# microsoft/OmniParser

Hardware: AMD Instinct MI355X
Metric: screenshots/sec end-to-end (detect+caption) @1920x1080 (higher is better)
Workload: dtype f32 (split-f16x3 MFMA)

## Files before the change

### include/omni_amd.h

```cpp
#ifndef OMNI_AMD_H
#define OMNI_AMD_H

#include <stdint.h>
#include <stddef.h>

#ifdef __cplusplus
extern "C" {
#endif

#define OMNI_ABI_VERSION 3

enum { OMNI_F32 = 0, OMNI_F16 = 1 };
enum { OMNI_ACT_NONE = 0, OMNI_ACT_SILU = 1, OMNI_ACT_GELU = 2 };
enum {
  OMNI_OK = 0,
  OMNI_E_ARG = -1,
  OMNI_E_HIP = -2,
  OMNI_E_NODEV = -3
};

const char* omni_last_error(void);
int omni_abi_version(void);
int omni_device_count(void);
int omni_overflow_count(int reset, unsigned long long* count);
// ... 46 lines not shown

#define OMNI_VOCAB_HEADER_BYTES 32
#define OMNI_VOCAB_MAX_NODES 65536
#define OMNI_VOCAB_MAX_LABEL 64
typedef struct omni_vocab_trie {
  int32_t n_nodes;
  int32_t n_edges;
  int32_t longest;
  int32_t reserved[5];
} omni_vocab_trie_t;

#define OMNI_GEN_CTRL_HEADER_BYTES 32
#define OMNI_GEN_CTRL_MAX_BAD 64
#define OMNI_GEN_CTRL_MAX_BAD_LEN 8
typedef struct omni_gen_ctrl {
  float penalty;
  int32_t ngram;
  int32_t min_new_tokens;
  int32_t begin_index;
  int32_t n_bad;
  int32_t bad_stride;
  int32_t reserved[2];
} omni_gen_ctrl_t;

typedef struct omni_cand {
  float x1, y1, x2, y2;
  float score;
  int32_t cls;
  int32_t anchor;
  int32_t pad;
} omni_cand_t;

int omni_op_launch(const omni_op_t* op, void* stream);

typedef struct omni_plan omni_plan_t;
int omni_plan_create(const omni_op_t* ops, int n_ops, omni_plan_t** out);
int omni_plan_run(omni_plan_t* plan, void* stream);
int omni_plan_capture(omni_plan_t* plan, void* stream);
int omni_plan_replay(omni_plan_t* plan, void* stream);
int omni_plan_num_ops(const omni_plan_t* plan);
void omni_plan_destroy(omni_plan_t* plan);

int omni_resample_coeffs(int in_size, int out_size, int filter, int32_t* h_bounds, int32_t* h_coef);

int omni_plan_time(omni_plan_t* plan, void* stream, int iters, float* ms);

int omni_plan_profile(omni_plan_t* plan, void* stream, float* h_ms);

int omni_debug_tile_map(int mtiles, int ntiles, int xcd_n, long long weight_bytes, int bid, int* mt, int* nt, int* grid,
                        int* xcd_n_used);

int omni_debug_conv_cfg(const omni_op_t* op, int out[8]);

int omni_visual_match_cfg(const omni_op_t* op, long long out[4]);

typedef struct omni_model omni_model_t;

int  omni_model_load(const char* bundle_path, omni_model_t** out);
void omni_model_destroy(omni_model_t* model);
int  omni_model_int(const omni_model_t* model, const char* name, long long* value);
int  omni_model_tensor(const omni_model_t* model, const char* name, void** d_ptr, long long* nbytes);
int  omni_model_run(omni_model_t* model, const char* plan_name);

int  omni_detector_create(const char* bundle_path, omni_model_t** out);
int  omni_detector_infer(omni_model_t* det, const uint8_t* images_rgb, int n_images, int on_device, float* h_boxes, float* h_scores,
                         int32_t* h_classes, int32_t* h_counts);

int  omni_captioner_create(const char* bundle_path, omni_model_t** out);
int  omni_captioner_caption(omni_model_t* cap, const uint8_t* image_rgb, int on_device, int img_h, int img_w, const int32_t* h_boxes_px,
                            int n, int32_t* h_ids);

#ifdef __cplusplus
}
#endif
#endif
```

### omniparser_amd/_lib.py

```python
import ctypes
from ctypes import c_char_p, c_float, c_int, c_int32, c_void_p, POINTER, Structure

from . import build as _build


F32, F16 = 0, 1
ACT_NONE, ACT_SILU, ACT_GELU = 0, 1, 2
OP_CONV, OP_AVGPOOL2, OP_MAXPOOL, OP_RESIZE_NEAREST, OP_LETTERBOX, OP_DETECT_DECODE, OP_NMS = 1, 2, 3, 4, 5, 6, 7
OP_DWCONV3, OP_LAYERNORM, OP_ATTN_ROWS, OP_CHAN_ATTN, OP_PROJ_PREP, OP_ASSEMBLE = 8, 9, 10, 11, 12, 13
OP_EMBED_STEP, OP_ATTN_DECODE, OP_GREEDY_STEP, OP_CROP_RESIZE, OP_DWCONV3_LN, OP_SPLIT_CONVERT, OP_GLUE = 14, 15, 16, 17, 18, 19, 20
OP_OVERLAY, OP_PNG_PACK, OP_PNG_DEFLATE, OP_MLP_FUSED, OP_BEAM_STEP = 21, 22, 23, 24, 25
OP_GREEDY_CTRL_STEP = 26
OP_GREEDY_VOCAB_STEP = 27
OP_VISUAL_MATCH = 28
OP_REGION_OCR = 29
OCR_CLASS_STRIP, OCR_CLASS_TEXT, OCR_CLASS_HARD = 1000, 1001, 1002
CAND_BYTES = 32
ABI_VERSION = 3

EXPORTS = [
    "omni_last_error", "omni_abi_version", "omni_device_count", "omni_op_launch",
    "omni_plan_create", "omni_plan_run", "omni_plan_capture", "omni_plan_replay",
    "omni_plan_num_ops", "omni_plan_destroy", "omni_resample_coeffs", "omni_plan_time", "omni_debug_tile_map",
    "omni_debug_conv_cfg",
    "omni_plan_profile",
    "omni_model_load", "omni_model_destroy", "omni_model_int", "omni_model_tensor", "omni_model_run",
    "omni_detector_create", "omni_detector_infer", "omni_captioner_create", "omni_captioner_caption",
    "omni_overflow_count",
    "omni_visual_match_cfg",
]


class OmniOp(Structure):
    _fields_ = [
        ("kind", c_int32),
        ("dtype", c_int32),
        ("p", c_void_p * 8),
        ("i", c_int32 * 32),
        ("f", c_float * 8),
    ]


class OmniError(RuntimeError):
    pass


_lib = None


def lib():
    global _lib
    if _lib is not None:
        return _lib
    path = _build.ensure_built()
    import torch
    _lib = bind(path)
    return _lib


def bind(path):
    L = ctypes.CDLL(str(path))
    missing = [s for s in EXPORTS if not hasattr(L, s)]
    if missing:
        raise OmniError(f"{path} does not export {missing}")
    L.omni_last_error.restype = c_char_p
    L.omni_abi_version.restype = c_int
    L.omni_device_count.restype = c_int
    L.omni_op_launch.argtypes = [POINTER(OmniOp), c_void_p]
    L.omni_op_launch.restype = c_int
    L.omni_plan_create.argtypes = [POINTER(OmniOp), c_int, POINTER(c_void_p)]
    L.omni_plan_create.restype = c_int
    for name in ("omni_plan_run", "omni_plan_capture", "omni_plan_replay"):
        fn = getattr(L, name)
        fn.argtypes = [c_void_p, c_void_p]
        fn.restype = c_int
    L.omni_plan_num_ops.argtypes = [c_void_p]
    L.omni_plan_num_ops.restype = c_int
    L.omni_plan_destroy.argtypes = [c_void_p]
    L.omni_plan_destroy.restype = None
    L.omni_resample_coeffs.argtypes = [c_int, c_int, c_int, POINTER(c_int32), POINTER(c_int32)]
    L.omni_resample_coeffs.restype = c_int
    L.omni_plan_time.argtypes = [c_void_p, c_void_p, c_int, POINTER(c_float)]
    L.omni_plan_time.restype = c_int
    L.omni_plan_profile.argtypes = [c_void_p, c_void_p, POINTER(c_float)]
    L.omni_plan_profile.restype = c_int
    L.omni_debug_tile_map.argtypes = [c_int, c_int, c_int, ctypes.c_longlong, c_int, POINTER(c_int), POINTER(c_int), POINTER(c_int),
                                      POINTER(c_int)]
    L.omni_debug_tile_map.restype = c_int
    L.omni_debug_conv_cfg.argtypes = [POINTER(OmniOp), POINTER(c_int)]
    L.omni_debug_conv_cfg.restype = c_int
    c_ll = ctypes.c_longlong
    for name in ("omni_model_load", "omni_detector_create", "omni_captioner_create"):
        fn = getattr(L, name)
        fn.argtypes = [c_char_p, POINTER(c_void_p)]
        fn.restype = c_int
    L.omni_model_destroy.argtypes = [c_void_p]
    L.omni_model_destroy.restype = None
    L.omni_model_int.argtypes = [c_void_p, c_char_p, POINTER(c_ll)]
    L.omni_model_int.restype = c_int
    L.omni_model_tensor.argtypes = [c_void_p, c_char_p, POINTER(c_void_p), POINTER(c_ll)]
    L.omni_model_tensor.restype = c_int
    L.omni_model_run.argtypes = [c_void_p, c_char_p]
    L.omni_model_run.restype = c_int
    L.omni_detector_infer.argtypes = [c_void_p, c_void_p, c_int, c_int, POINTER(c_float), POINTER(c_float), POINTER(c_int32), POINTER(c_int32)]
    L.omni_detector_infer.restype = c_int
    L.omni_captioner_caption.argtypes = [c_void_p, c_void_p, c_int, c_int, c_int, POINTER(c_int32), c_int, POINTER(c_int32)]
    L.omni_captioner_caption.restype = c_int
    L.omni_overflow_count.argtypes = [c_int, POINTER(ctypes.c_ulonglong)]
    L.omni_overflow_count.restype = c_int
    L.omni_visual_match_cfg.argtypes = [POINTER(OmniOp), POINTER(ctypes.c_longlong)]
    L.omni_visual_match_cfg.restype = c_int
    if L.omni_abi_version() != ABI_VERSION:
        raise OmniError(f"ABI version mismatch: library {L.omni_abi_version()}, host code {ABI_VERSION} (rebuild: python -m omniparser_amd.build)")
    return L


def overflow_count(reset=True) -> int:
    n = ctypes.c_ulonglong(0)
    rc = lib().omni_overflow_count(1 if reset else 0, ctypes.byref(n))
    if rc:
        raise OmniError(lib().omni_last_error().decode())
    return int(n.value)


def gc_after_eviction():
    import gc
    if gc.get_freeze_count():
        gc.unfreeze()
        gc.collect()
        gc.freeze()


def require_device(device, what):
    import torch
    device = torch.device(device or ("cuda" if torch.cuda.is_available() else "cpu"))
    if device.type == "cuda" and not torch.cuda.is_available():
        raise RuntimeError(f"CUDA device requested but unavailable: {device}")
    if device.type != "cuda":
        raise RuntimeError(f"omniparser_amd {what} is the MI355X path and has no CPU fallback; use the reference implementation on CPU")
    if device.index is None:
        device = torch.device("cuda", torch.cuda.current_device())
    return device

# ... 91 lines not shown
        return ms.value

    def profile(self, stream=None):
        arr = (c_float * len(self.ops))()
        check(lib().omni_plan_profile(self._h, _stream_ptr(stream), arr))
        return list(arr)

    def __len__(self):
        return len(self.ops)

    def __del__(self):
        try:
            if self._h:
                lib().omni_plan_destroy(self._h)
                self._h = None
        except Exception:
            pass


def resample_coeffs(in_size: int, out_size: int, filt: int):
    import numpy as np
    k = lib().omni_resample_coeffs(in_size, out_size, filt, None, None)
    if k <= 0:
        check(k)
    bounds = np.zeros((out_size, 2), dtype=np.int32)
    coef = np.zeros((out_size, k), dtype=np.int32)
    rc = lib().omni_resample_coeffs(
        in_size, out_size, filt,
        bounds.ctypes.data_as(POINTER(c_int32)), coef.ctypes.data_as(POINTER(c_int32)))
    if rc <= 0:
        check(rc)
    return bounds, coef


def tile_map(mtiles: int, ntiles: int, bid: int, xcd_n: int = 1, weight_bytes: int = -1):
    mt, nt, grid, used = c_int(), c_int(), c_int(), c_int()
    check(lib().omni_debug_tile_map(mtiles, ntiles, xcd_n, weight_bytes, bid, ctypes.byref(mt), ctypes.byref(nt), ctypes.byref(grid),
                                    ctypes.byref(used)))
    return mt.value, nt.value, grid.value, used.value


CONV_FAMILIES = ("f32", "f16", "split")
CONV_LOADERS = ("generic", "aligned", "pointwise", "row_patch")
CONV_REDUCE = ("none", "reduce_launch", "in_launch_combine")


def conv_cfg(op: OmniOp) -> dict:
    out = (c_int * 8)()
    check(lib().omni_debug_conv_cfg(ctypes.byref(op), out))
    return {"family": CONV_FAMILIES[out[0]], "bm": out[1], "bn": out[2], "rb": out[3], "loader": CONV_LOADERS[out[4]],
            "splits": out[5], "reduce": CONV_REDUCE[out[6]], "waves": out[7]}


class CModel:

    def __init__(self, path, kind):
        h = c_void_p()
        fn = {"detector": lib().omni_detector_create, "captioner": lib().omni_captioner_create, "model": lib().omni_model_load}[kind]
        check(fn(str(path).encode(), ctypes.byref(h)))
        self._h, self.kind = h, kind

    def int(self, name):
        v = ctypes.c_longlong()
        check(lib().omni_model_int(self._h, name.encode(), ctypes.byref(v)))
        return v.value

    def infer(self, images_u8):
        import numpy as np
        n, md = images_u8.shape[0], self.int("max_det")
        im = np.ascontiguousarray(images_u8)
        boxes = np.zeros((n, md, 4), np.float32); scores = np.zeros((n, md), np.float32)
        cls = np.zeros((n, md), np.int32); cnt = np.zeros((n,), np.int32)
        check(lib().omni_detector_infer(self._h, im.ctypes.data_as(c_void_p), n, 0, boxes.ctypes.data_as(POINTER(c_float)),
                                        scores.ctypes.data_as(POINTER(c_float)), cls.ctypes.data_as(POINTER(c_int32)),
                                        cnt.ctypes.data_as(POINTER(c_int32))))
        return boxes, scores, cls, cnt

    def caption(self, image_u8, boxes_px):
        import numpy as np
        im = np.ascontiguousarray(image_u8)
        bx = np.ascontiguousarray(np.asarray(boxes_px, dtype=np.int32).reshape(-1, 4))
        ids = np.zeros((bx.shape[0], self.int("T")), np.int32)
        check(lib().omni_captioner_caption(self._h, im.ctypes.data_as(c_void_p), 0, im.shape[0], im.shape[1],
                                           bx.ctypes.data_as(POINTER(c_int32)), bx.shape[0], ids.ctypes.data_as(POINTER(c_int32))))
        return ids

    def tensor(self, name):
        p, n = c_void_p(), ctypes.c_longlong()
        check(lib().omni_model_tensor(self._h, name.encode(), ctypes.byref(p), ctypes.byref(n)))
        return p.value, n.value

    def close(self):
        if self._h:
            lib().omni_model_destroy(self._h)
            self._h = None

    def __del__(self):
        try:
            self.close()
        except Exception:
            pass
```

### omniparser_amd/csrc/caption_ops.hip

```cpp
#include "omni_internal.h"
#include <stdlib.h>

#pragma clang fp contract(off)

OMNI_RANGE_GUARD_TU()

namespace {

template <typename T> __device__ __forceinline__ float ldf(const T* p) { return ElemTraits<T>::to_f32(*p); }
template <typename T> __device__ __forceinline__ void stf(T* p, float v) { *p = ElemTraits<T>::from_f32(v); }

__device__ __forceinline__ float wave_sum(float v) {
#pragma unroll
  for (int o = 32; o > 0; o >>= 1) v += __shfl_xor(v, o);
  return v;
}
__device__ __forceinline__ float wave_max(float v) {
#pragma unroll
  for (int o = 32; o > 0; o >>= 1) v = fmaxf(v, __shfl_xor(v, o));
  return v;
}

struct DwArgs { const void* x; const void* w; const float* bias; void* y; int B, H, W, C; long long total; };

template <typename T>
__host__ __device__ __forceinline__ void dwconv3_point_body(const DwArgs& a, long long idx) {
  constexpr int V = ElemTraits<T>::kVec;
  struct Vec { T v[V]; };
  const T* __restrict__ X = (const T*)a.x;
  const T* __restrict__ Wt = (const T*)a.w;
  T* __restrict__ Y = (T*)a.y;
  const int cv = a.C / V;
  int c = (int)(idx % cv) * V;
  long long pix = idx / cv;
  int w = (int)(pix % a.W);
  long long t = pix / a.W;
  int h = (int)(t % a.H);
  long long b = t / a.H;
  float acc[V];
#pragma unroll
  for (int e = 0; e < V; ++e) acc[e] = 0.0f;
  Vec ctr;
#pragma unroll
  for (int r = 0; r < 3; ++r) {
    int hi = h + r - 1;
    if (hi < 0 || hi >= a.H) continue;
#pragma unroll
    for (int s = 0; s < 3; ++s) {
      int wi = w + s - 1;
      if (wi < 0 || wi >= a.W) continue;
      Vec xv = __builtin_bit_cast(Vec, *reinterpret_cast<const u32x4*>(X + ((b * a.H + hi) * a.W + wi) * a.C + c));
      Vec wv = __builtin_bit_cast(Vec, *reinterpret_cast<const u32x4*>(Wt + (r * 3 + s) * a.C + c));
      if (r == 1 && s == 1) ctr = xv;
#pragma unroll
// ... 346 lines not shown
  load_row(h0, r1);
  load_row(h0 + 1, r2);
  const float invC = 1.0f / (float)a.C;
  for (int h = h0; h < h1; ++h) {
    if (h + 1 < h1) load_row(h + 2, nx);
    f32x4 y[NV];
    float s = 0.0f;
#pragma unroll
    for (int i = 0; i < NV; ++i) {
      f32x4 acc = z4;
#pragma unroll
      for (int q = 0; q < 3; ++q) acc += wt[0 + q][i] * r0[q][i];
#pragma unroll
      for (int q = 0; q < 3; ++q) acc += wt[3 + q][i] * r1[q][i];
#pragma unroll
      for (int q = 0; q < 3; ++q) acc += wt[6 + q][i] * r2[q][i];
      y[i] = (acc + cb[i]) + r1[1][i];
      s += (y[i][0] + y[i][1]) + (y[i][2] + y[i][3]);
    }
    const long long pix = (long long)h * a.W + w;
#pragma unroll
    for (int i = 0; i < NV; ++i) *reinterpret_cast<f32x4*>(Y1 + pix * a.C + (l + i * LPP) * 4) = y[i];
    const float mean = group_sum<LPP>(s) * invC;
    float q2 = 0.0f;
#pragma unroll
    for (int i = 0; i < NV; ++i) {
      const f32x4 d = y[i] - mean;
      q2 += (d[0] * d[0] + d[1] * d[1]) + (d[2] * d[2] + d[3] * d[3]);
    }
    const float rstd = 1.0f / sqrtf(group_sum<LPP>(q2) * invC + a.eps);
#pragma unroll
    for (int i = 0; i < NV; ++i) {
      const int c = (l + i * LPP) * 4;
      float o[4];
#pragma unroll
      for (int e = 0; e < 4; ++e) o[e] = (y[i][e] - mean) * rstd * lg[i][e] + lb[i][e];
      if constexpr (OSPLIT) {
        uint2 hi, lo;
        omni_split4(o, hi, lo);
        unsigned char* p = Hh + pix * a.C * 4 + omni_split_off(c);
        *reinterpret_cast<uint2*>(p) = hi;
        *reinterpret_cast<uint2*>(p + 32) = lo;
      } else {
        *reinterpret_cast<f32x4*>(Hh + (pix * a.C + c) * 4) = f32x4{o[0], o[1], o[2], o[3]};
      }
    }
#pragma unroll
    for (int q = 0; q < 3; ++q)
#pragma unroll
      for (int i = 0; i < NV; ++i) { r0[q][i] = r1[q][i]; r1[q][i] = r2[q][i]; r2[q][i] = nx[q][i]; }
  }
}

template <int NV, int LPP>
void launch_dwln_strip(const DwLnArgs& a, hipStream_t s) {
  constexpr int PPB = 256 / LPP;
  const int pxb = (a.W + PPB - 1) / PPB;
  int SR = 16;
  while (SR > 4 && (long long)a.B * ((a.H + SR - 1) / SR) * pxb < 1024) SR >>= 1;
  const int strips = (a.H + SR - 1) / SR;
  const long long nb = (long long)a.B * strips * pxb;
  const unsigned grid = (unsigned)(((nb + 7) / 8) * 8);
  if (a.osplit) hipLaunchKernelGGL((dwln_strip_kernel<NV, LPP, true>), dim3(grid), dim3(256), 0, s, a, SR, pxb, strips, (unsigned)nb);
  else hipLaunchKernelGGL((dwln_strip_kernel<NV, LPP, false>), dim3(grid), dim3(256), 0, s, a, SR, pxb, strips, (unsigned)nb);
}

struct AttnArgs {
  const void* q; const void* k; const void* v; void* o; const float* kbias; const float* vbias;
  int ldq, ldk, ldv, ldo, qoff, koff, voff, ooff;
  int heads, nq, nk, groups;
  int mode, H, W, wy, wx;
  float scale;
  int osplit;
  const int* nkeys;
};

__device__ __forceinline__ int attn_valid_keys(const AttnArgs& a, int g) {
  return a.nkeys ? min(max(a.nkeys[g], 1), a.nk) : a.nk;
}

template <typename T>
__device__ __forceinline__ void store_out(void* base, long long row, int ld, int c, float v, int osplit) {
  if (osplit) {
    unsigned short hi, lo;
    omni_split1(v, hi, lo);
    unsigned short* p = (unsigned short*)base + row * ld * 2 + omni_split_half_index(c);
    p[0] = hi;
    p[16] = lo;
  } else {
    stf((T*)base + row * ld + c, v);
  }
}

__device__ __forceinline__ long long window_row(const AttnArgs& a, int g, int i) {
  int wpi = a.wy * a.wx;
  int b = g / wpi, wrem = g - b * wpi;
  int wyi = wrem / a.wx, wxi = wrem - wyi * a.wx;
  int r = wyi * 12 + i / 12, c = wxi * 12 + i % 12;
  if (r >= a.H || c >= a.W) return -1;
  return ((long long)b * a.H + r) * a.W + c;
}

template <typename T, int D, int NT>
__global__ __launch_bounds__(NT) void attn_rows_kernel(AttnArgs a) {
  constexpr int KT = 48;
  __shared__ __attribute__((aligned(16))) float sk[KT][D];
  __shared__ __attribute__((aligned(16))) float sv[KT][D];
  const int g = blockIdx.z, h = blockIdx.y;
  const int qi = blockIdx.x * NT + threadIdx.x;
  const T* Q = (const T*)a.q; const T* K = (const T*)a.k; const T* V = (const T*)a.v;
  long long qrow = -1;
  if (qi < a.nq) qrow = a.mode == 1 ? window_row(a, g, qi) : (long long)g * a.nq + qi;
  float q[D], o[D];
#pragma unroll
// ... 197 lines not shown
#pragma unroll
      for (int dt = 0; dt < 2; ++dt) {
        const unsigned char* vr = Vh + (dt * 16 + qc) * VROW + (32 * j + 4 * grp) * 2;
        h16x4 a0 = *reinterpret_cast<const h16x4*>(vr), a1 = *reinterpret_cast<const h16x4*>(vr + 32);
        h16x4 b0 = *reinterpret_cast<const h16x4*>(vr + D * VROW), b1 = *reinterpret_cast<const h16x4*>(vr + D * VROW + 32);
        h16x8 vh = {a0[0], a0[1], a0[2], a0[3], a1[0], a1[1], a1[2], a1[3]};
        h16x8 vl = {b0[0], b0[1], b0[2], b0[3], b1[0], b1[1], b1[2], b1[3]};
        oM[dt] = __builtin_amdgcn_mfma_f32_16x16x32_f16(ph, vh, oM[dt], 0, 0, 0);
        oC[dt] = __builtin_amdgcn_mfma_f32_16x16x32_f16(ph, vl, oC[dt], 0, 0, 0);
        oC[dt] = __builtin_amdgcn_mfma_f32_16x16x32_f16(pl, vh, oC[dt], 0, 0, 0);
      }
    }
#pragma unroll
    for (int r = 0; r < 4; ++r) {
      int ql_ = grp * 4 + r;
      float rs = __shfl(sum, ql_);
      long long orow = window_row(a, g, qt * 16 + ql_);
      if (orow >= 0) {
        float inv = 1.0f / rs;
#pragma unroll
        for (int dt = 0; dt < 2; ++dt)
          store_out<T>(a.o, orow, a.ldo, a.ooff + h * D + dt * 16 + qc, (oM[dt][r] + oC[dt][r] * inv2048) * inv, a.osplit);
      }
    }
  }
}

__device__ __forceinline__ void split2(float a, float b, unsigned& h, unsigned& l) {
  typedef __fp16 hv2 __attribute__((ext_vector_type(2)));
  const hv2 hh = __builtin_amdgcn_cvt_pkrtz(a, b);
  const f32x2 r = (f32x2{a, b} - f32x2{(float)hh[0], (float)hh[1]}) * 2048.0f;
  const hv2 ll = __builtin_amdgcn_cvt_pkrtz(r[0], r[1]);
  h = __builtin_bit_cast(unsigned, hh);
  l = __builtin_bit_cast(unsigned, ll);
}
__device__ __forceinline__ void split4v(const f32x4& v, uint2& h, uint2& l) {
  split2(v[0], v[1], h.x, l.x);
  split2(v[2], v[3], h.y, l.y);
}

__device__ __forceinline__ void split2m(float a, float b, unsigned& h, unsigned& l) {
  typedef __fp16 hv2 __attribute__((ext_vector_type(2)));
  const hv2 hh = __builtin_amdgcn_cvt_pkrtz(a, b);
  const f32x2 s = f32x2{a, b} * 2048.0f;
  const hv2 ll = __builtin_amdgcn_cvt_pkrtz(__builtin_fmaf((float)hh[0], -2048.0f, s[0]), __builtin_fmaf((float)hh[1], -2048.0f, s[1]));
  h = __builtin_bit_cast(unsigned, hh);
  l = __builtin_bit_cast(unsigned, ll);
}
__device__ __forceinline__ void split4m(const f32x4& v, uint2& h, uint2& l) {
  split2m(v[0], v[1], h.x, l.x);
  split2m(v[2], v[3], h.y, l.y);
}

__global__ __launch_bounds__(192, 2) void window_attn_mfma_f32_kernel(AttnArgs a) {
  constexpr int D = 32, NKP = 160, KROW = 80, VROW = 336;
  __shared__ __attribute__((aligned(16))) unsigned char lds[2 * NKP * KROW + 2 * D * VROW];
  unsigned char* Kh = lds;
  unsigned char* Kl = lds + NKP * KROW;
  unsigned char* Vh = lds + 2 * NKP * KROW;
  unsigned char* Vl = Vh + D * VROW;
  const int g = blockIdx.z, h = blockIdx.y;
  const int tid = threadIdx.x, lane = tid & 63, wave = tid >> 6;
  const int wpi = a.wy * a.wx;
  const int b = g / wpi, wrem = g - b * wpi;
  const int wyi = wrem / a.wx, wxi = wrem - wyi * a.wx;
  const int r0 = wyi * 12, c0 = wxi * 12;
  const int rows_left = a.H - r0, cols_left = a.W - c0;
  const long long row00 = ((long long)b * a.H + r0) * a.W + c0;
  const float* Qb = (const float*)a.q + row00 * a.ldq + a.qoff + h * D;
  const float* Kb = (const float*)a.k + row00 * a.ldk + a.koff + h * D;
  const float* Vb = (const float*)a.v + row00 * a.ldv + a.voff + h * D;
  const int qc = lane & 15, grp = lane >> 4;
  const f32x4 z4 = {0.f, 0.f, 0.f, 0.f};
  const int iq0 = 16 * wave + qc;
  const int qwr = iq0 / 12, qwc = iq0 - 12 * qwr;
  const int qtok = qwr * a.W + qwc;
  f32x4 qraw[3][2];
#pragma unroll
  for (int t = 0; t < 3; ++t) {
    const bool ok = qwr + 4 * t < rows_left && qwc < cols_left;
    const float* qp = Qb + (ok ? (qtok + 4 * t * a.W) * a.ldq : 0) + grp * 8;
    qraw[t][0] = ok ? *reinterpret_cast<const f32x4*>(qp) : z4;
    qraw[t][1] = ok ? *reinterpret_cast<const f32x4*>(qp + 4) : z4;
  }
  const int t8 = tid >> 3, d0 = (tid & 7) * 4;
  const int kwr = t8 >= 12 ? 1 : 0, kwc = t8 - 12 * kwr;
  const int ktok = kwr * a.W + kwc;
  f32x4 kpad = z4, vpad = z4;
  if (a.kbias) kpad = *reinterpret_cast<const f32x4*>(a.kbias + h * D + d0);
  if (a.vbias) vpad = *reinterpret_cast<const f32x4*>(a.vbias + h * D + d0);
  f32x4 kraw[6];
#pragma unroll
  for (int j = 0; j < 6; ++j) {
    const bool ok = kwr + 2 * j < rows_left && kwc < cols_left;
    kraw[j] = ok ? *reinterpret_cast<const f32x4*>(Kb + (ktok + 2 * j * a.W) * a.ldk + d0) : kpad;
  }
  const int vwr = t8 / 3, vwc = 4 * (t8 - 3 * vwr);
  const int vtok = vwr * a.W + vwc;
  f32x4 vraw[2][4];
#pragma unroll
  for (int j = 0; j < 2; ++j) {
    if (j == 0 || tid < 96) {
#pragma unroll
      for (int u = 0; u < 4; ++u) {
        const bool ok = vwr + 8 * j < rows_left && vwc + u < cols_left;
        vraw[j][u] = ok ? *reinterpret_cast<const f32x4*>(Vb + (vtok + 8 * j * a.W + u) * a.ldv + d0) : vpad;
      }
    }
  }
#pragma unroll
  for (int j = 0; j < 6; ++j) {
    const int key = t8 + 24 * j;
    uint2 kh, kl;
    split4m(kraw[j], kh, kl);
    *reinterpret_cast<uint2*>(Kh + key * KROW + d0 * 2) = kh;
    *reinterpret_cast<uint2*>(Kl + key * KROW + d0 * 2) = kl;
  }
  if (tid >= 128) {
    const int r = tid - 128;
    unsigned char* p = (r < 32 ? Vh : Vl) + (r & 31) * VROW + 144 * 2;
    const u32x4 z = {0u, 0u, 0u, 0u};
    *reinterpret_cast<u32x4*>(p) = z;
    *reinterpret_cast<u32x4*>(p + 16) = z;
  }
#pragma unroll
  for (int j = 0; j < 2; ++j) {
    const int kq = t8 + 24 * j;
    if (j == 0 || tid < 96) {
#pragma unroll
      for (int dd = 0; dd < 4; ++dd) {
        uint2 vh, vl;
        split4m(f32x4{vraw[j][0][dd], vraw[j][1][dd], vraw[j][2][dd], vraw[j][3][dd]}, vh, vl);
        *reinterpret_cast<uint2*>(Vh + (d0 + dd) * VROW + kq * 8) = vh;
        *reinterpret_cast<uint2*>(Vl + (d0 + dd) * VROW + kq * 8) = vl;
      }
    }
  }
  __syncthreads();

  const float inv2048 = 1.0f / 2048.0f;
  const float qscale = a.scale * 1.4426950408889634f;
  unsigned char* const Ob = (unsigned char*)a.o + (row00 * a.ldo + a.ooff + h * D) * 4;
#pragma unroll
  for (int t = 0; t < 3; ++t) {
    u32x4 qhu, qlu;
    {
      const f32x4 q0 = qraw[t][0] * qscale, q1 = qraw[t][1] * qscale;
      uint2 h0, l0, h1, l1;
      split4m(q0, h0, l0);
      split4m(q1, h1, l1);
      qhu = u32x4{h0.x, h0.y, h1.x, h1.y};
      qlu = u32x4{l0.x, l0.y, l1.x, l1.y};
    }
    const h16x8 qh = __builtin_bit_cast(h16x8, qhu), ql = __builtin_bit_cast(h16x8, qlu);
    f32x2 sc[18];
    float mx = -INFINITY;
#pragma unroll
    for (int kt = 0; kt < 9; ++kt) {
      const unsigned char* kr = Kh + (kt * 16 + qc) * KROW + grp * 16;
      const h16x8 kh = *reinterpret_cast<const h16x8*>(kr);
      const h16x8 kl = *reinterpret_cast<const h16x8*>(kr + NKP * KROW);
      f32x4 accM = z4, accC = z4;
      accM = __builtin_amdgcn_mfma_f32_16x16x32_f16(kh, qh, accM, 0, 0, 0);
      accC = __builtin_amdgcn_mfma_f32_16x16x32_f16(kh, ql, accC, 0, 0, 0);
      accC = __builtin_amdgcn_mfma_f32_16x16x32_f16(kl, qh, accC, 0, 0, 0);
      sc[2 * kt] = f32x2{accC[0], accC[1]} * inv2048 + f32x2{accM[0], accM[1]};
      sc[2 * kt + 1] = f32x2{accC[2], accC[3]} * inv2048 + f32x2{accM[2], accM[3]};
      mx = fmaxf(fmaxf(mx, sc[2 * kt][0]), sc[2 * kt][1]);
      mx = fmaxf(fmaxf(mx, sc[2 * kt + 1][0]), sc[2 * kt + 1][1]);
    }
    mx = fmaxf(mx, __shfl_xor(mx, 16));
    mx = fmaxf(mx, __shfl_xor(mx, 32));
    f32x2 sum2 = {0.f, 0.f};
#pragma unroll
    for (int e = 0; e < 18; ++e) {
      const f32x2 d = sc[e] - mx;
      sc[e] = f32x2{__builtin_amdgcn_exp2f(d[0]), __builtin_amdgcn_exp2f(d[1])};
      sum2 += sc[e];
    }
    float sum = sum2[0] + sum2[1];
    sum += __shfl_xor(sum, 16);
    sum += __shfl_xor(sum, 32);
    f32x4 oM[2], oC[2];
#pragma unroll
    for (int dt = 0; dt < 2; ++dt) { oM[dt] = z4; oC[dt] = z4; }
#pragma unroll
    for (int j = 0; j < 5; ++j) {
      unsigned h0, l0, h1, l1, h2 = 0u, l2 = 0u, h3 = 0u, l3 = 0u;
      split2m(sc[4 * j][0], sc[4 * j][1], h0, l0);
      split2m(sc[4 * j + 1][0], sc[4 * j + 1][1], h1, l1);
      if (j < 4) {
        split2m(sc[4 * j + 2][0], sc[4 * j + 2][1], h2, l2);
        split2m(sc[4 * j + 3][0], sc[4 * j + 3][1], h3, l3);
      }
      const h16x8 ph = __builtin_bit_cast(h16x8, u32x4{h0, h1, h2, h3});
      const h16x8 pl = __builtin_bit_cast(h16x8, u32x4{l0, l1, l2, l3});
#pragma unroll
      for (int dt = 0; dt < 2; ++dt) {
        const unsigned char* vr = Vh + (dt * 16 + qc) * VROW + (32 * j + 4 * grp) * 2;
        const uint2 a0 = *reinterpret_cast<const uint2*>(vr), a1 = *reinterpret_cast<const uint2*>(vr + 32);
        const uint2 b0 = *reinterpret_cast<const uint2*>(vr + D * VROW), b1 = *reinterpret_cast<const uint2*>(vr + D * VROW + 32);
        const h16x8 vh = __builtin_bit_cast(h16x8, u32x4{a0.x, a0.y, a1.x, a1.y});
        const h16x8 vl = __builtin_bit_cast(h16x8, u32x4{b0.x, b0.y, b1.x, b1.y});
        oM[dt] = __builtin_amdgcn_mfma_f32_16x16x32_f16(vh, ph, oM[dt], 0, 0, 0);
        oC[dt] = __builtin_amdgcn_mfma_f32_16x16x32_f16(vl, ph, oC[dt], 0, 0, 0);
        oC[dt] = __builtin_amdgcn_mfma_f32_16x16x32_f16(vh, pl, oC[dt], 0, 0, 0);
      }
    }
    if (qwr + 4 * t < rows_left && qwc < cols_left) {
      const float inv = 1.0f / sum;
      unsigned char* orow = Ob + (long long)(qtok + 4 * t * a.W) * a.ldo * 4;
#pragma unroll
      for (int dt = 0; dt < 2; ++dt) {
        const f32x4 o = (oC[dt] * inv2048 + oM[dt]) * inv;
        const int c = dt * 16 + 4 * grp;
        if (a.osplit) {
          const float v[4] = {o[0], o[1], o[2], o[3]};
          uint2 hi, lo;
          omni_split4(v, hi, lo);
          *reinterpret_cast<uint2*>(orow + omni_split_off(c)) = hi;
          *reinterpret_cast<uint2*>(orow + omni_split_off(c) + 32) = lo;
        } else {
          *reinterpret_cast<f32x4*>(orow + c * 4) = o;
        }
      }
    }
  }
}

template <typename T>
__global__ __launch_bounds__(256, 2) void mha_mfma_kernel(AttnArgs a) {
  constexpr int D = 64, KB = 32;
  constexpr int KROW = 144;
  constexpr int VROW = 80;
  __shared__ __attribute__((aligned(16))) unsigned char lds[2 * KB * KROW + 2 * D * VROW];
  unsigned char* Kh = lds;
  unsigned char* Kl = lds + KB * KROW;
  unsigned char* Vh = lds + 2 * KB * KROW;
  unsigned char* Vl = Vh + D * VROW;
  const int g = blockIdx.z, h = blockIdx.y;
  const int tid = threadIdx.x, lane = tid & 63, wave = tid >> 6;
  const int qc = lane & 15, grp = lane >> 4;
  const T* Qp = (const T*)a.q; const T* Kp = (const T*)a.k; const T* Vp = (const T*)a.v;
  const float inv2048 = 1.0f / 2048.0f;

  const int q0 = blockIdx.x * 128 + wave * 32;
  h16x8 qh[2][2], ql[2][2];
#pragma unroll
  for (int t = 0; t < 2; ++t) {
    int qi = q0 + t * 16 + qc;
#pragma unroll
    for (int ks = 0; ks < 2; ++ks) {
#pragma unroll
      for (int u = 0; u < 8; ++u) {
// ... 1593 lines not shown
    for (int y = 0; y < cnt; ++y) {
      const unsigned char* s = a.tmp + (((long long)crop * 64 + ymin + y) * a.R + xx) * 3;
      int kk = k[y]; s0 += s[0] * kk; s1 += s[1] * kk; s2 += s[2] * kk;
    }
    p[0] = clip8b(s0); p[1] = clip8b(s1); p[2] = clip8b(s2);
  }
  T* out = (T*)a.y + ((long long)crop * a.R * a.R + idx) * a.ldo;
#pragma unroll
  for (int c = 0; c < 3; ++c) {
    float v = a.lut[p[c]];
    stf(out + c, (v - a.mean[c]) / a.stdv[c]);
  }
  for (int c = 3; c < a.ldo; ++c) stf(out + c, 0.0f);
}

template <typename F32, typename F16>
int by_dtype(int dtype, const char* name, F32 f32, F16 f16) {
  if (dtype == OMNI_F32) f32();
  else if (dtype == OMNI_F16) f16();
  else { omni_set_error("%s: bad dtype %d", name, dtype); return OMNI_E_ARG; }
  return OMNI_OK;
}

template <typename L>
int by_dtype_scores(int dtype, bool scores, const char* name, L launch) {
  return scores ? by_dtype(dtype, name, [&] { launch(float{}, std::true_type{}); }, [&] { launch(half_t{}, std::true_type{}); })
                : by_dtype(dtype, name, [&] { launch(float{}, std::false_type{}); }, [&] { launch(half_t{}, std::false_type{}); });
}

}

int omni_launch_dwconv3(const omni_op_t* op, hipStream_t s) {
  DwArgs a{};
  a.x = op->p[0]; a.w = op->p[1]; a.bias = (const float*)op->p[2]; a.y = op->p[4];
  a.B = op->i[0]; a.H = op->i[1]; a.W = op->i[2]; a.C = op->i[3];
  OMNI_REQUIRE(a.x && a.w && a.bias && a.y && a.B > 0 && a.H > 0 && a.W > 0 && a.C > 0, "dwconv3: bad arguments");
  OMNI_REQUIRE(a.C % (op->dtype == OMNI_F32 ? 4 : 8) == 0, "dwconv3: C must be a multiple of the 16-byte vector width");
  a.total = (long long)a.B * a.H * a.W * a.C;
  const int V = op->dtype == OMNI_F32 ? 4 : 8;
  const DwStripGrid g = dwconv3_strip_grid(a, V);
  int rc;
  if (g.ok) {
    rc = by_dtype(op->dtype, "dwconv3",
        [&] { hipLaunchKernelGGL(dwconv3_strip_kernel<float>, dim3(g.gx, g.gy, g.gz), dim3(256), 0, s, a, g.cv_log2); },
        [&] { hipLaunchKernelGGL(dwconv3_strip_kernel<half_t>, dim3(g.gx, g.gy, g.gz), dim3(256), 0, s, a, g.cv_log2); });
  } else {
    long long blocks = (a.total / V + 255) / 256; if (blocks > 65536) blocks = 65536;
    rc = by_dtype(op->dtype, "dwconv3",
        [&] { hipLaunchKernelGGL(dwconv3_kernel<float>, dim3((unsigned)blocks), dim3(256), 0, s, a); },
        [&] { hipLaunchKernelGGL(dwconv3_kernel<half_t>, dim3((unsigned)blocks), dim3(256), 0, s, a); });
  }
  if (rc) return rc;
  OMNI_HIP_CHECK(hipGetLastError());
  return OMNI_OK;
}

int omni_launch_dwconv3_ln(const omni_op_t* op, hipStream_t s) {
  DwLnArgs a{};
  a.x = op->p[0]; a.w = op->p[1]; a.bias = (const float*)op->p[2]; a.h = op->p[3]; a.y1 = op->p[4];
  a.g = (const float*)op->p[5]; a.b = (const float*)op->p[6];
  a.B = op->i[0]; a.H = op->i[1]; a.W = op->i[2]; a.C = op->i[3]; a.eps = op->f[0]; a.osplit = op->i[6];
  const int V = op->dtype == OMNI_F32 ? 4 : 8;
  OMNI_REQUIRE(a.x && a.w && a.bias && a.h && a.y1 && a.g && a.b, "dwconv3_ln: null pointer");
  OMNI_REQUIRE(!a.osplit || (op->dtype == OMNI_F32 && a.C % 16 == 0), "dwconv3_ln: split output needs an f32 plan and C %% 16 == 0");
  OMNI_REQUIRE(a.B > 0 && a.H > 0 && a.W > 0 && a.C > 0 && a.C <= 1024 && a.C % V == 0, "dwconv3_ln: bad shape (C <= 1024, C %% %d == 0)", V);
  a.pixels = (long long)a.B * a.H * a.W;
  if (op->dtype == OMNI_F32 && (a.C == 128 || a.C == 256 || a.C == 512) && (long long)a.B * a.H * a.W < (1ll << 31)) {
    if (a.C == 128) launch_dwln_strip<1, 32>(a, s);
    else if (a.C == 256) launch_dwln_strip<1, 64>(a, s);
    else launch_dwln_strip<2, 64>(a, s);
    OMNI_HIP_CHECK(hipGetLastError());
    return OMNI_OK;
  }
  unsigned blocks = (unsigned)((a.pixels + 3) / 4);
  int rc = by_dtype(op->dtype, "dwconv3_ln",
      [&] { hipLaunchKernelGGL(dwconv3_ln_kernel<float>, dim3(blocks), dim3(256), 0, s, a); },
      [&] { hipLaunchKernelGGL(dwconv3_ln_kernel<half_t>, dim3(blocks), dim3(256), 0, s, a); });
  if (rc) return rc;
  OMNI_HIP_CHECK(hipGetLastError());
  return OMNI_OK;
}

int omni_launch_layernorm(const omni_op_t* op, hipStream_t s) {
  LnArgs a{};
  a.x = op->p[0]; a.add = op->p[1]; a.g = (const float*)op->p[2]; a.b = (const float*)op->p[3]; a.y = op->p[4];
  a.rows = ((long long)op->i[0]) * (op->i[1] > 0 ? op->i[1] : 1); a.C = op->i[3]; a.period = op->i[5] > 0 ? op->i[5] : 1;
  a.eps = op->f[0];
  a.omode = op->i[6]; a.y2 = op->p[5];
  OMNI_REQUIRE(a.x && a.g && a.b && a.y && a.rows > 0 && a.C > 0 && a.C <= 1024, "layernorm: bad arguments (C <= 1024)");
  OMNI_REQUIRE(a.omode >= 0 && a.omode <= 2 && (a.omode != 2 || a.y2), "layernorm: bad output mode %d", a.omode);
  OMNI_REQUIRE(a.omode == 0 || (op->dtype == OMNI_F32 && a.C % 16 == 0), "layernorm: split output needs an f32 plan and C %% 16 == 0");
  if (op->dtype == OMNI_F32 && launch_layernorm_v4(a, s)) {
    OMNI_HIP_CHECK(hipGetLastError());
    return OMNI_OK;
  }
  unsigned blocks = (unsigned)((a.rows + 3) / 4);
  int rc = by_dtype(op->dtype, "layernorm",
      [&] { launch_layernorm_typed<float>(a, blocks, s); },
      [&] { launch_layernorm_typed<half_t>(a, blocks, s); });
  if (rc) return rc;
  OMNI_HIP_CHECK(hipGetLastError());
  return OMNI_OK;
}

static int launch_attn_rows(const omni_op_t* op, hipStream_t s) {
  AttnArgs a{};
  a.q = op->p[0]; a.k = op->p[1]; a.v = op->p[2]; a.o = op->p[4];
  a.kbias = (const float*)op->p[5]; a.vbias = (const float*)op->p[6];
  a.ldq = op->i[0]; a.ldk = op->i[1]; a.ldv = op->i[2]; a.ldo = op->i[3];
  a.qoff = op->i[4]; a.koff = op->i[5]; a.voff = op->i[6]; a.ooff = op->i[7];
  a.heads = op->i[8]; a.nq = op->i[9]; a.nk = op->i[10]; a.groups = op->i[11];
  a.mode = op->i[12]; a.H = op->i[13]; a.W = op->i[14];
  int D = op->i[15];
  a.scale = op->f[0];
  a.osplit = op->i[16];
  a.nkeys = (const int*)op->p[7];
  OMNI_REQUIRE(a.q && a.k && a.v && a.o && a.heads > 0 && a.nq > 0 && a.nk > 0 && a.groups > 0, "attn_rows: bad arguments");
  OMNI_REQUIRE(!a.nkeys || a.mode == 0, "attn_rows: the per-group key count (p7) is for mode 0");
  OMNI_REQUIRE(!a.osplit || (op->dtype == OMNI_F32 && a.ldo % 16 == 0 && a.ooff % 16 == 0), "attn_rows: split output needs an f32 plan, 16-channel aligned");
  OMNI_REQUIRE(D == 32 || D == 64, "attn_rows: head_dim %d unsupported", D);
  if (a.mode == 1) {
    OMNI_REQUIRE(a.nq == 144 && a.nk == 144 && a.H > 0 && a.W > 0, "attn_rows: window mode needs 12x12 windows");
    a.wy = (a.H + 11) / 12; a.wx = (a.W + 11) / 12;
    OMNI_REQUIRE(a.groups % (a.wy * a.wx) == 0, "attn_rows: groups must be B * windows");
  } else { a.wy = a.wx = 0; }
  int rc;
  const bool aligned4 = a.ldq % 4 == 0 && a.ldk % 4 == 0 && a.ldv % 4 == 0 && a.ldo % 4 == 0 &&
                        a.qoff % 4 == 0 && a.koff % 4 == 0 && a.voff % 4 == 0 && a.ooff % 4 == 0;
  OMNI_REQUIRE(!a.osplit || (a.mode == 1 && D == 32) || (a.mode == 0 && D == 64), "attn_rows: split output exists on the MFMA kernels only");
  if (a.mode == 1 && D == 32) {
    dim3 grid(1, a.heads, a.groups);
    OMNI_REQUIRE(op->dtype != OMNI_F32 || aligned4, "attn_rows: the f32 window kernel reads 16-byte rows (pitches and channel offsets %% 4 == 0)");
    rc = by_dtype(op->dtype, "attn_rows",
      [&] { hipLaunchKernelGGL(window_attn_mfma_f32_kernel, grid, dim3(192), 0, s, a); },
      [&] { hipLaunchKernelGGL((window_attn_mfma_kernel<half_t>), grid, dim3(192), 0, s, a); });
  } else if (a.mode == 0 && D == 64) {
    dim3 grid((a.nq + 127) / 128, a.heads, a.groups);
    OMNI_REQUIRE(op->dtype != OMNI_F32 || aligned4, "attn_rows: the f32 MHA kernel reads 16-byte rows (pitches and channel offsets %% 4 == 0)");
    rc = by_dtype(op->dtype, "attn_rows",
      [&] { hipLaunchKernelGGL(mha_mfma_f32_kernel, grid, dim3(256), 0, s, a); },
      [&] { hipLaunchKernelGGL((mha_mfma_kernel<half_t>), grid, dim3(256), 0, s, a); });
  } else {
    dim3 grid((a.nq + 127) / 128, a.heads, a.groups);
    if (D == 32) rc = by_dtype(op->dtype, "attn_rows",
      [&] { hipLaunchKernelGGL((attn_rows_kernel<float, 32, 128>), grid, dim3(128), 0, s, a); },
      [&] { hipLaunchKernelGGL((attn_rows_kernel<half_t, 32, 128>), grid, dim3(128), 0, s, a); });
    else rc = by_dtype(op->dtype, "attn_rows",
      [&] { hipLaunchKernelGGL((attn_rows_kernel<float, 64, 128>), grid, dim3(128), 0, s, a); },
      [&] { hipLaunchKernelGGL((attn_rows_kernel<half_t, 64, 128>), grid, dim3(128), 0, s, a); });
  }
  if (rc) return rc;
  OMNI_HIP_CHECK(hipGetLastError());
  return OMNI_OK;
}

int omni_launch_chan_repack(const omni_op_t* op, hipStream_t s) {
  FoldArgs f{};
  const int B = op->i[0], C = op->i[3];
  f.wf = (float*)op->p[0]; f.wb = (unsigned char*)op->p[4]; f.bmax = (float*)op->p[5]; f.osc = (float*)op->p[6];
  OMNI_REQUIRE(op->dtype == OMNI_F32 && f.wf && f.wb && f.bmax && f.osc, "split_convert (i6 = 1): f32 plans, p0 / p4 / p5 / p6");
  OMNI_REQUIRE(B > 0 && C > 0 && C % 64 == 0 && op->i[1] == C && op->i[4] == C && op->i[5] == 0 && op->i[13] == C && op->i[14] == 0,
               "split_convert (i6 = 1): i0 square matrices of i1 = i3 = i4 = i13 = C, C %% 64 == 0, no channel offsets (C %d)", C);
  f.C = C; f.G = C / 32; f.nblk = (C / 64) * (C / 32); f.oscmul = 1.0f;
  hipLaunchKernelGGL(chan_fold_max_kernel, dim3(f.nblk, B), dim3(256), 0, s, f);
  hipLaunchKernelGGL(chan_fold_pack_kernel, dim3((C * (C / 16) + 255) / 256, B), dim3(256), 0, s, f);
  OMNI_HIP_CHECK(hipGetLastError());
  return OMNI_OK;
}

static int launch_chan_attn(const omni_op_t* op, hipStream_t s) {
  ChanArgs a{};
  a.qkv = op->p[0]; a.o = op->p[4]; a.ws = (float*)op->p[5];
  a.B = op->i[0]; a.N = op->i[1]; a.C = op->i[3]; a.G = op->i[4]; a.chunk_tokens = op->i[5]; a.osplit = op->i[6];
  const bool fold = op->i[8] == 1;
  OMNI_REQUIRE(a.qkv && (a.o || fold) && a.ws && a.B > 0 && a.N > 0 && a.C == a.G * 32 && a.chunk_tokens > 0, "chan_attn: bad arguments");
  OMNI_REQUIRE(op->i[8] == 0 || fold, "chan_attn: unknown mode %d", op->i[8]);
  OMNI_REQUIRE(!fold || (op->dtype == OMNI_F32 && a.chunk_tokens % 8 == 0 && a.C % 64 == 0 && op->p[1] && op->p[2] && op->p[3] && op->p[6] && op->p[7]),
               "chan_attn: fold mode needs an f32 plan, C %% 64 == 0, chunk_tokens %% 8 == 0 and p1 / p2 / p3 / p6 / p7");
  OMNI_REQUIRE(!a.osplit || op->dtype == OMNI_F32, "chan_attn: split output needs an f32 plan");
  const int vfold = op->i[11];
  OMNI_REQUIRE(vfold == 0 || (vfold == 1 && fold && a.C % 128 == 0), "chan_attn: i11 = %d needs fold mode (i8 = 1) and C %% 128 == 0, and is 0 or 1", vfold);
  const bool have_scores = op->i[9] == 1;
  if (op->i[10] != 0) {
    OMNI_REQUIRE(op->i[10] > 0 && op->i[10] % 8 == 0 && a.chunk_tokens % op->i[10] == 0 && op->dtype == OMNI_F32 && a.C % 4 == 0,
                 "chan_attn: i10 = %d (tokens per partial) needs an f32 plan, i10 %% 8 == 0 and i5 %% i10 == 0", op->i[10]);
    a.chunk_tokens = op->i[10];
  }
// ... 244 lines not shown
```

Before: 12.91.

## Swizzle window-attention LDS layout and pick dwconv-LN strip height by cost

The f32 window-attention kernel gets a new default LDS layout: K and V split images are XOR-swizzled instead of padded. This shrinks shared memory so three blocks per CU fit instead of two, and it drops the zero-fill of the V pad. Separately, the dwconv3+LN strip launcher for C=128 now picks the strip height from a cost model that uses occupancy-derived slot counts, rather than the fixed 16-row rule. Env vars can force the old paths, and a debug export reports the strip choice. The risks are bank-conflict regressions from the swizzle and extra conditional V reads in the last key chunk.

```diff
diff --git a/include/omni_amd.h b/include/omni_amd.h
--- a/include/omni_amd.h
+++ b/include/omni_amd.h
@@ -122,6 +122,8 @@
 
 int omni_debug_conv_cfg(const omni_op_t* op, int out[8]);
 
+int omni_debug_dwln_sr(const omni_op_t* op, int slots, int out[8]);
+
 int omni_visual_match_cfg(const omni_op_t* op, long long out[4]);
 
 typedef struct omni_model omni_model_t;
diff --git a/omniparser_amd/_lib.py b/omniparser_amd/_lib.py
--- a/omniparser_amd/_lib.py
+++ b/omniparser_amd/_lib.py
@@ -22,7 +22,7 @@
     "omni_last_error", "omni_abi_version", "omni_device_count", "omni_op_launch",
     "omni_plan_create", "omni_plan_run", "omni_plan_capture", "omni_plan_replay",
     "omni_plan_num_ops", "omni_plan_destroy", "omni_resample_coeffs", "omni_plan_time", "omni_debug_tile_map",
-    "omni_debug_conv_cfg",
+    "omni_debug_conv_cfg", "omni_debug_dwln_sr",
     "omni_plan_profile",
     "omni_model_load", "omni_model_destroy", "omni_model_int", "omni_model_tensor", "omni_model_run",
     "omni_detector_create", "omni_detector_infer", "omni_captioner_create", "omni_captioner_caption",
@@ -89,6 +89,8 @@
     L.omni_debug_tile_map.restype = c_int
     L.omni_debug_conv_cfg.argtypes = [POINTER(OmniOp), POINTER(c_int)]
     L.omni_debug_conv_cfg.restype = c_int
+    L.omni_debug_dwln_sr.argtypes = [POINTER(OmniOp), c_int, POINTER(c_int)]
+    L.omni_debug_dwln_sr.restype = c_int
     c_ll = ctypes.c_longlong
     for name in ("omni_model_load", "omni_detector_create", "omni_captioner_create"):
         fn = getattr(L, name)
@@ -286,6 +288,13 @@
             "splits": out[5], "reduce": CONV_REDUCE[out[6]], "waves": out[7]}
 
 
+def dwln_sr(op: OmniOp, slots: int) -> dict:
+    out = (c_int * 8)()
+    check(lib().omni_debug_dwln_sr(ctypes.byref(op), slots, out))
+    return {"sr": out[0], "strips": out[1], "blocks": out[2], "cost_sr": out[3], "cost_rounds": out[4], "cost": out[5],
+            "how": ("rule16", "cost", "forced")[out[6]], "cols_per_block": out[7]}
+
+
 class CModel:
 
     def __init__(self, path, kind):
diff --git a/omniparser_amd/csrc/caption_ops.hip b/omniparser_amd/csrc/caption_ops.hip
--- a/omniparser_amd/csrc/caption_ops.hip
+++ b/omniparser_amd/csrc/caption_ops.hip
@@ -1,5 +1,6 @@
 #include "omni_internal.h"
 #include <stdlib.h>
+#include <string.h>
 
 #pragma clang fp contract(off)
 
@@ -452,14 +453,69 @@
   }
 }
 
+struct DwlnStripCfg { int SR, strips; long long nb; int cost_SR; long long cost_rounds, cost; int how; };
+
+static long long dwln_strip_cost(int B, int H, int pxb, int SR, int slots, long long* rounds) {
+  const int rows = SR < H ? SR : H, strips = (H + rows - 1) / rows;
+  const long long nb = (long long)B * strips * pxb;
+  *rounds = (nb + slots - 1) / slots;
+  const int loaded = rows + (strips == 1 ? 0 : strips == 2 ? 1 : 2);
+  return *rounds * (loaded + 2 * rows);
+}
+
+static bool dwln_cost_adopted(int C) { return C == 128; }
+
+static DwlnStripCfg dwln_strip_cfg(const DwLnArgs& a, int pxb, int slots) {
+  DwlnStripCfg c{};
+  c.cost_SR = 0;
+  if (slots > 0) {
+    const int cand[7] = {8, 16, 24, 32, 48, 96, a.H};
+    for (int k = 0; k < 7; ++k) {
+      if (cand[k] > a.H) continue;
+      long long r;
+      const long long cost = dwln_strip_cost(a.B, a.H, pxb, cand[k], slots, &r);
+      if (!c.cost_SR || cost <= c.cost) { c.cost_SR = cand[k]; c.cost = cost; c.cost_rounds = r; }
+    }
+  }
+  const char* e = getenv("OMNI_DWLN_SR");
+  const bool want_cost = e && !strcmp(e, "cost");
+  const int forced = (e && !want_cost) ? atoi(e) : 0;
+  if (forced > 0) { c.SR = forced < a.H ? forced : a.H; c.how = 2; }
+  else if (c.cost_SR && (want_cost || dwln_cost_adopted(a.C))) { c.SR = c.cost_SR; c.how = 1; }
+  else {
+    c.SR = 16; c.how = 0;
+    while (c.SR > 4 && (long long)a.B * ((a.H + c.SR - 1) / c.SR) * pxb < 1024) c.SR >>= 1;
+  }
+  c.strips = (a.H + c.SR - 1) / c.SR;
+  c.nb = (long long)a.B * c.strips * pxb;
+  return c;
+}
+
+template <int NV, int LPP>
+int dwln_strip_slots() {
+#if defined(__HIP__)
+  static const int slots = [] {
+    int per_cu = 0, dev = 0, cus = 0;
+    if (hipOccupancyMaxActiveBlocksPerMultiprocessor(&per_cu, dwln_strip_kernel<NV, LPP, true>, 256, 0) != hipSuccess ||
+        hipGetDevice(&dev) != hipSuccess || hipDeviceGetAttribute(&cus, hipDeviceAttributeMultiprocessorCount, dev) != hipSuccess) {
+      (void)hipGetLastError();
+      return 0;
+    }
+    return per_cu > 0 && cus > 0 ? per_cu * cus : 0;
+  }();
+  return slots;
+#else
+  return 0;
+#endif
+}
+
 template <int NV, int LPP>
 void launch_dwln_strip(const DwLnArgs& a, hipStream_t s) {
   constexpr int PPB = 256 / LPP;
   const int pxb = (a.W + PPB - 1) / PPB;
-  int SR = 16;
-  while (SR > 4 && (long long)a.B * ((a.H + SR - 1) / SR) * pxb < 1024) SR >>= 1;
-  const int strips = (a.H + SR - 1) / SR;
-  const long long nb = (long long)a.B * strips * pxb;
+  const DwlnStripCfg cfg = dwln_strip_cfg(a, pxb, dwln_strip_slots<NV, LPP>());
+  const int SR = cfg.SR, strips = cfg.strips;
+  const long long nb = cfg.nb;
   const unsigned grid = (unsigned)(((nb + 7) / 8) * 8);
   if (a.osplit) hipLaunchKernelGGL((dwln_strip_kernel<NV, LPP, true>), dim3(grid), dim3(256), 0, s, a, SR, pxb, strips, (unsigned)nb);
   else hipLaunchKernelGGL((dwln_strip_kernel<NV, LPP, false>), dim3(grid), dim3(256), 0, s, a, SR, pxb, strips, (unsigned)nb);
@@ -763,13 +819,34 @@
   split2m(v[2], v[3], h.y, l.y);
 }
 
-__global__ __launch_bounds__(192, 2) void window_attn_mfma_f32_kernel(AttnArgs a) {
-  constexpr int D = 32, NKP = 160, KROW = 80, VROW = 336;
-  __shared__ __attribute__((aligned(16))) unsigned char lds[2 * NKP * KROW + 2 * D * VROW];
+template <bool PADDED> struct WinLds;
+template <> struct WinLds<true> {
+  static constexpr int KIMG = 160 * 80, VIMG = 32 * 336;
+  static __device__ __forceinline__ int k_store(int key, int d0) { return key * 80 + d0 * 2; }
+  static __device__ __forceinline__ int k_read(int kt, int qc, int grp) { return (kt * 16 + qc) * 80 + grp * 16; }
+  static __device__ __forceinline__ int v_chunk(int ch, int c, int lo) { return lo * VIMG + ch * 336 + c * 8; }
+};
+template <> struct WinLds<false> {
+  static constexpr int KIMG = 144 * 64, VIMG = 9 * 1024;
+  static __device__ __forceinline__ int kswz(int key) { return (-(key >> 2)) & 3; }
+  static __device__ __forceinline__ int k_store(int key, int d0) { return key * 64 + (((d0 >> 3) ^ kswz(key)) << 4) + ((d0 & 4) << 1); }
+  static __device__ __forceinline__ int k_read(int kt, int qc, int grp) { return (kt * 16 + qc) * 64 + ((grp ^ kswz(qc)) << 4); }
+  static __device__ __forceinline__ int v_chunk(int ch, int c, int lo) {
+    const int vrow = ((ch >> 2) & 3) | ((ch & 3) << 2) | (ch & 16), vswz = (ch & 1) | ((((ch >> 1) ^ (ch >> 4)) & 1) << 1);
+    const int kb = c >> 2, blk = kb < 8 ? lo * 8 + kb : 16 + lo;
+    return blk * 1024 + vrow * 32 + (((c & 3) ^ vswz) << 3);
+  }
+};
+
+template <bool PADDED>
+__global__ __launch_bounds__(192, PADDED ? 2 : 3) void window_attn_mfma_f32_kernel(AttnArgs a) {
+  constexpr int D = 32;
+  constexpr int KIMG = WinLds<PADDED>::KIMG, VIMG = WinLds<PADDED>::VIMG;
+  typedef WinLds<PADDED> Lds;
+  __shared__ __attribute__((aligned(16))) unsigned char lds[2 * KIMG + 2 * VIMG];
   unsigned char* Kh = lds;
-  unsigned char* Kl = lds + NKP * KROW;
-  unsigned char* Vh = lds + 2 * NKP * KROW;
-  unsigned char* Vl = Vh + D * VROW;
+  unsigned char* Kl = lds + KIMG;
+  unsigned char* V = lds + 2 * KIMG;
   const int g = blockIdx.z, h = blockIdx.y;
   const int tid = threadIdx.x, lane = tid & 63, wave = tid >> 6;
   const int wpi = a.wy * a.wx;
@@ -824,15 +901,18 @@
     const int key = t8 + 24 * j;
     uint2 kh, kl;
     split4m(kraw[j], kh, kl);
-    *reinterpret_cast<uint2*>(Kh + key * KROW + d0 * 2) = kh;
-    *reinterpret_cast<uint2*>(Kl + key * KROW + d0 * 2) = kl;
-  }
-  if (tid >= 128) {
-    const int r = tid - 128;
-    unsigned char* p = (r < 32 ? Vh : Vl) + (r & 31) * VROW + 144 * 2;
-    const u32x4 z = {0u, 0u, 0u, 0u};
-    *reinterpret_cast<u32x4*>(p) = z;
-    *reinterpret_cast<u32x4*>(p + 16) = z;
+    const int ko = Lds::k_store(key, d0);
+    *reinterpret_cast<uint2*>(Kh + ko) = kh;
+    *reinterpret_cast<uint2*>(Kl + ko) = kl;
+  }
+  if constexpr (PADDED) {
+    if (tid >= 128) {
+      const int r = tid - 128;
+      unsigned char* p = (r < 32 ? V : V + VIMG) + (r & 31) * 336 + 144 * 2;
+      const u32x4 z = {0u, 0u, 0u, 0u};
+      *reinterpret_cast<u32x4*>(p) = z;
+      *reinterpret_cast<u32x4*>(p + 16) = z;
+    }
   }
 #pragma unroll
   for (int j = 0; j < 2; ++j) {
@@ -842,8 +922,13 @@
       for (int dd = 0; dd < 4; ++dd) {
         uint2 vh, vl;
         split4m(f32x4{vraw[j][0][dd], vraw[j][1][dd], vraw[j][2][dd], vraw[j][3][dd]}, vh, vl);
-        *reinterpret_cast<uint2*>(Vh + (d0 + dd) * VROW + kq * 8) = vh;
-        *reinterpret_cast<uint2*>(Vl + (d0 + dd) * VROW + kq * 8) = vl;
+        if constexpr (PADDED) {
+          *reinterpret_cast<uint2*>(V + (d0 + dd) * 336 + kq * 8) = vh;
+          *reinterpret_cast<uint2*>(V + VIMG + (d0 + dd) * 336 + kq * 8) = vl;
+        } else {
+          *reinterpret_cast<uint2*>(V + Lds::v_chunk(d0 + dd, kq, 0)) = vh;
+          *reinterpret_cast<uint2*>(V + Lds::v_chunk(d0 + dd, kq, 1)) = vl;
+        }
       }
     }
   }
@@ -868,9 +953,9 @@
     float mx = -INFINITY;
 #pragma unroll
     for (int kt = 0; kt < 9; ++kt) {
-      const unsigned char* kr = Kh + (kt * 16 + qc) * KROW + grp * 16;
+      const unsigned char* kr = Kh + Lds::k_read(kt, qc, grp);
       const h16x8 kh = *reinterpret_cast<const h16x8*>(kr);
-      const h16x8 kl = *reinterpret_cast<const h16x8*>(kr + NKP * KROW);
+      const h16x8 kl = *reinterpret_cast<const h16x8*>(kr + KIMG);
       f32x4 accM = z4, accC = z4;
       accM = __builtin_amdgcn_mfma_f32_16x16x32_f16(kh, qh, accM, 0, 0, 0);
       accC = __builtin_amdgcn_mfma_f32_16x16x32_f16(kh, ql, accC, 0, 0, 0);
@@ -908,9 +993,21 @@
       const h16x8 pl = __builtin_bit_cast(h16x8, u32x4{l0, l1, l2, l3});
 #pragma unroll
       for (int dt = 0; dt < 2; ++dt) {
-        const unsigned char* vr = Vh + (dt * 16 + qc) * VROW + (32 * j + 4 * grp) * 2;
-        const uint2 a0 = *reinterpret_cast<const uint2*>(vr), a1 = *reinterpret_cast<const uint2*>(vr + 32);
-        const uint2 b0 = *reinterpret_cast<const uint2*>(vr + D * VROW), b1 = *reinterpret_cast<const uint2*>(vr + D * VROW + 32);
+        const int vr = dt * 16 + qc, c0 = 8 * j + grp, c1 = c0 + 4;
+        uint2 a0, a1, b0, b1;
+        if constexpr (PADDED) {
+          const unsigned char* vp = V + vr * 336 + c0 * 8;
+          a0 = *reinterpret_cast<const uint2*>(vp); a1 = *reinterpret_cast<const uint2*>(vp + 32);
+          b0 = *reinterpret_cast<const uint2*>(vp + VIMG); b1 = *reinterpret_cast<const uint2*>(vp + VIMG + 32);
+        } else {
+          a0 = *reinterpret_cast<const uint2*>(V + Lds::v_chunk(vr, c0, 0));
+          b0 = *reinterpret_cast<const uint2*>(V + Lds::v_chunk(vr, c0, 1));
+          a1 = b1 = uint2{0u, 0u};
+          if (j < 4) {
+            a1 = *reinterpret_cast<const uint2*>(V + Lds::v_chunk(vr, c1, 0));
+            b1 = *reinterpret_cast<const uint2*>(V + Lds::v_chunk(vr, c1, 1));
+          }
+        }
         const h16x8 vh = __builtin_bit_cast(h16x8, u32x4{a0.x, a0.y, a1.x, a1.y});
         const h16x8 vl = __builtin_bit_cast(h16x8, u32x4{b0.x, b0.y, b1.x, b1.y});
         oM[dt] = __builtin_amdgcn_mfma_f32_16x16x32_f16(vh, ph, oM[dt], 0, 0, 0);
@@ -2610,6 +2707,20 @@
   }
   if (rc) return rc;
   OMNI_HIP_CHECK(hipGetLastError());
+  return OMNI_OK;
+}
+
+extern "C" int omni_debug_dwln_sr(const omni_op_t* op, int slots, int out[8]) {
+  OMNI_REQUIRE(op && out, "omni_debug_dwln_sr: null argument");
+  OMNI_REQUIRE(op->kind == OMNI_OP_DWCONV3_LN && op->dtype == OMNI_F32 && (op->i[3] == 128 || op->i[3] == 256 || op->i[3] == 512),
+               "omni_debug_dwln_sr: not a strip-kernel op (f32, C = 128 / 256 / 512)");
+  DwLnArgs a{};
+  a.B = op->i[0]; a.H = op->i[1]; a.W = op->i[2]; a.C = op->i[3];
+  OMNI_REQUIRE(a.B > 0 && a.H > 0 && a.W > 0 && slots >= 0, "omni_debug_dwln_sr: bad shape");
+  const int PPB = a.C == 128 ? 8 : 4;
+  const DwlnStripCfg c = dwln_strip_cfg(a, (a.W + PPB - 1) / PPB, slots);
+  out[0] = c.SR; out[1] = c.strips; out[2] = (int)c.nb; out[3] = c.cost_SR; out[4] = (int)c.cost_rounds; out[5] = (int)c.cost;
+  out[6] = c.how; out[7] = PPB;
   return OMNI_OK;
 }
 
@@ -2689,8 +2800,14 @@
   if (a.mode == 1 && D == 32) {
     dim3 grid(1, a.heads, a.groups);
     OMNI_REQUIRE(op->dtype != OMNI_F32 || aligned4, "attn_rows: the f32 window kernel reads 16-byte rows (pitches and channel offsets %% 4 == 0)");
+    const char* lds_e = getenv("OMNI_WINDOW_ATTN_LDS");
+    const bool padded = lds_e && !strcmp(lds_e, "padded");
+    OMNI_REQUIRE(!lds_e || !lds_e[0] || padded || !strcmp(lds_e, "swizzled"), "attn_rows: OMNI_WINDOW_ATTN_LDS is 'padded' or 'swizzled', not '%s'", lds_e);
     rc = by_dtype(op->dtype, "attn_rows",
-      [&] { hipLaunchKernelGGL(window_attn_mfma_f32_kernel, grid, dim3(192), 0, s, a); },
+      [&] {
+        if (padded) hipLaunchKernelGGL((window_attn_mfma_f32_kernel<true>), grid, dim3(192), 0, s, a);
+        else hipLaunchKernelGGL((window_attn_mfma_f32_kernel<false>), grid, dim3(192), 0, s, a);
+      },
       [&] { hipLaunchKernelGGL((window_attn_mfma_kernel<half_t>), grid, dim3(192), 0, s, a); });
   } else if (a.mode == 0 && D == 64) {
     dim3 grid((a.nq + 127) / 128, a.heads, a.groups);
```

After: 12.94, median of 6. Within noise of the previous version (+0.2%).
